# Deci-AI/super-gradients

Hardware: AMD Instinct MI355X
Metric: images/sec/node YOLO-NAS-S 640x640 train-step (higher is better)
Workload: dtype fp32 (bf16x3 MFMA); 1 GPU; YOLO-NAS-S synthetic COCO 640x640, bs=32/GPU, PPYoloELoss(TAL)+AdamW+EMA, random-init weights; global_batch=32, parallelism=dp1, conv_math=patch_bf3, conv_variant=0, bn_reduce_in_data_gradients=True, conv_tuning_entries=374, filter_planes=True

## Files before the change

### include/sgx_hip.h

```cpp
#ifndef SGX_HIP_H
#define SGX_HIP_H
#include <stdint.h>

#ifdef __cplusplus
extern "C" {
#endif

#define SGX_OK 0
#define SGX_ERR_BAD_ARG (-1)
#define SGX_ERR_UNSUPPORTED (-2)
#define SGX_ERR_HIP (-3)
#define SGX_ERR_WORKSPACE (-4)

#define SGX_ACT_NONE 0
#define SGX_ACT_RELU 1
#define SGX_ACT_SILU 2

int32_t sgx_version(void);
const char* sgx_last_error(void);

int32_t sgx_prof_enable(int32_t on);
int32_t sgx_prof_summary(int32_t cls, double* ms, double* flops, int64_t* launches);
int32_t sgx_prof_bytes(int32_t cls, double* bytes);
int32_t sgx_prof_bound_ms(int32_t cls, double peak_flops, double hbm_bytes_per_s, double* ms);
// ... 153 lines not shown
int32_t sgx_affine_act_fwd(const float* x, int64_t x_ld, const float* scale, const float* shift, const float* r1,
                           int64_t r1_ld, float a1, const float* a1_dev, const float* r2, int64_t r2_ld, float a2,
                           float* y, int64_t y_ld, int64_t M, int32_t C, int32_t act, float* partials, void* stream);
int32_t sgx_bn_bwd_reduce(const float* dy, int64_t dy_ld, const float* x, int64_t x_ld, const float* scale,
                          const float* shift, const float* save_mean, int64_t M, int32_t C, int32_t act, float* partials,
                          void* stream);
int32_t sgx_bn_bwd_finalize(const float* partials, int32_t nblk, int64_t M, int32_t C, const float* gamma,
                            const float* save_mean, const float* save_invstd, float* dgamma, float* dbeta,
                            float* coef, void* ws, int64_t ws_bytes, void* stream);
int32_t sgx_bn_bwd_apply(const float* dy, int64_t dy_ld, const float* x, int64_t x_ld, const float* scale,
                         const float* shift, const float* coef, float* dx, int64_t dx_ld, float* g_out, int64_t g_ld,
                         int64_t M, int32_t C, int32_t act, void* stream);
int64_t sgx_qarep_workspace(int32_t nblk, int32_t C);
int32_t sgx_qarep_fwd_finalize(const float* stat5, int32_t nblk, int64_t M, int32_t C, const float* bias1, const float* gamma3, const float* beta3,
                               float eps3, float mom3, float* rmean3, float* rvar3, const float* gammap, const float* betap, float epsp, float momp,
                               float* rmeanp, float* rvarp, float* cf, float* sv, void* ws, int64_t ws_bytes, void* stream);
int32_t sgx_qarep_bwd_reduce(const float* dout, int64_t d_ld, const float* y, int64_t y_ld, const float* u, int64_t u_ld, const float* cf,
                             const float* sv, int64_t M, int32_t C, int32_t act, float* partials4, void* stream);
int32_t sgx_qarep_bwd_finalize(const float* partials4, int32_t nblk, int64_t M, int32_t C, const float* gamma3, const float* gammap, const float* sv,
                               float* dgamma3, float* dgammap, float* dbetap, float* cb, void* ws, int64_t ws_bytes, void* stream);
int32_t sgx_qarep_bwd_apply(const float* dout, int64_t d_ld, const float* y, int64_t y_ld, const float* u, int64_t u_ld, const float* cf,
                            const float* sv, const float* cb, float* ds, int64_t ds_ld, float* dy, int64_t dy_ld, int64_t M, int32_t C, int32_t act,
                            void* stream);
int32_t sgx_bn_set_fused_finalize(int32_t on);
int32_t sgx_bn_get_fused_finalize(void);
int64_t sgx_dot_workspace(int64_t M, int32_t C);
int32_t sgx_dot(const float* a, int64_t a_ld, const float* b, int64_t b_ld, int64_t M, int32_t C, float scale, float* out,
                int32_t accumulate, void* ws, int64_t ws_bytes, void* stream);
int32_t sgx_axpy(const float* x, int64_t x_ld, float a, const float* a_dev, float* y, int64_t y_ld, int64_t M,
                 int32_t C, int32_t accumulate, void* stream);
int32_t sgx_relu_bwd(const float* dy, int64_t dy_ld, const float* y, int64_t y_ld, float* g, int64_t g_ld, int64_t M, int32_t C,
                     void* stream);
int32_t sgx_relu_bwd_bn_reduce(const float* dy, int64_t dy_ld, const float* y, int64_t y_ld, const float* x, int64_t x_ld,
                               const float* save_mean, float* g, int64_t g_ld, int64_t M, int32_t C, float* partials, void* stream);
int32_t sgx_dual_affine_act_fwd(const float* x1, int64_t x1_ld, const float* s1, const float* t1, const float* x2, int64_t x2_ld,
                                const float* s2, const float* t2, const float* r, int64_t r_ld, float r_scale, const float* r_scale_dev,
                                float* y, int64_t y_ld, int64_t M, int32_t C, int32_t act, void* stream);
int32_t sgx_dual_affine_act_bwd(const float* dy, int64_t dy_ld, const float* x1, int64_t x1_ld, const float* s1, const float* t1,
                                const float* x2, int64_t x2_ld, const float* s2, const float* t2, float* g, int64_t g_ld, int64_t M,
                                int32_t C, int32_t act, void* stream);
int32_t sgx_dual_affine_act_bwd_reduce(const float* dy, int64_t dy_ld, const float* x1, int64_t x1_ld, const float* s1, const float* t1,
                                       const float* mean1, const float* x2, int64_t x2_ld, const float* s2, const float* t2, const float* mean2,
                                       float* g, int64_t g_ld, int64_t M, int32_t C, int32_t act, float* partials4, void* stream);
int32_t sgx_tri_affine_act_fwd(const float* x1, int64_t x1_ld, const float* s1, const float* t1, const float* x2, int64_t x2_ld,
                               const float* s2, const float* t2, const float* x3, int64_t x3_ld, const float* s3, const float* t3,
                               const float* r, int64_t r_ld, float r_scale, const float* r_scale_dev, float* y, int64_t y_ld, int64_t M,
// ... 148 lines not shown
```

### super_gradients_amd/_lib.py

```python
import ctypes
import os
from ctypes import POINTER, c_char_p, c_float, c_int32, c_int64, c_void_p

import torch

_HERE = os.path.dirname(os.path.abspath(__file__))
LIB_PATH = os.path.join(_HERE, "csrc", "libsgx_hip.so")

_LIB = None
_TEST_HOST_MODE = False


class ConvDesc(ctypes.Structure):
    _fields_ = [(n, c_int32) for n in ("N", "H", "W", "C", "K", "R", "S", "stride", "pad", "Ho", "Wo")] + [
        (n, c_int64) for n in ("x_ld_pix", "x_ld_img", "y_ld_pix", "y_ld_img")
    ]


class LossDesc(ctypes.Structure):
    _fields_ = [
        ("B", c_int32), ("L", c_int32), ("C", c_int32), ("reg_max", c_int32), ("nmax", c_int32),
        ("use_static_assigner", c_int32), ("use_varifocal", c_int32), ("num_levels", c_int32),
        ("level_count", c_int32 * 8), ("w_cls", c_float), ("w_iou", c_float), ("w_dfl", c_float), ("sequential_assignment", c_int32),
    ]
# ... 60 lines not shown
    "sgx_conv2d_bwd_data": (_i32, [_CD, _P, _P, _P, _P, _i32, _P, _i64, _P]),
    "sgx_conv2d_transpose_weights": (_i32, [_CD, _P, _P, _i64, _P]),
    "sgx_conv2d_bwd_data_wt": (_i32, [_CD, _P, _P, _P, _P, _i32, _P]),
    "sgx_conv2d_bwd_data_stat_blocks": (_i32, [_CD, _i32]),
    "sgx_conv2d_bwd_data_wt_req": (_i32, [_CD, _P, _P, _P, _P, _i32, POINTER(BnReduceReq), _i32, _P]),
    "sgx_conv2d_bwd_data_dual_req": (_i32, [_CD, _P, _P, _P, _i64, _i64, _P, _P, _P, _i64, _i64, _f, _P, _P, _i32, POINTER(BnReduceReq), _i32, _P]),
    "sgx_conv2d_transpose_jobs": (_i32, [_CD, _P, _P, _i64, POINTER(WtransJob), _i32, POINTER(c_int32)]),
    "sgx_wtrans_batch": (_i32, [_P, _i32, _P]),
    "sgx_conv2d_fwd_dual_stat_blocks": (_i32, [_CD]),
    "sgx_conv2d_fwd_dual": (_i32, [_CD, _P, _P, _P, _P, _P, _P, _P, _P]),
    "sgx_conv2d_bwd_data_dual": (_i32, [_CD, _P, _P, _P, _i64, _i64, _P, _P, _P, _i64, _i64, _f, _P, _P, _i32, _P]),
    "sgx_qarep_prep_batch": (_i32, [_P, _i32, _P]),
    "sgx_filter_planes_bytes": (_i64, [_i32, _i32, _i32]),
    "sgx_filter_planes_batch": (_i32, [_P, _P, _i32, _P]),
    "sgx_filter_planes_invalidate": (_i32, [_P, _i32]),
    "sgx_filter_planes_scope": (_i32, [_i32]),
    "sgx_debug_set_filter_planes": (_i32, [_i32]),
    "sgx_debug_filter_planes_hits": (_i64, []),
    "sgx_qarep_workspace": (_i64, [_i32, _i32]),
    "sgx_qarep_fwd_finalize": (_i32, [_P, _i32, _i64, _i32, _P, _P, _P, _f, _f, _P, _P, _P, _P, _f, _f, _P, _P, _P, _P, _P, _i64, _P]),
    "sgx_qarep_bwd_reduce": (_i32, [_P, _i64, _P, _i64, _P, _i64, _P, _P, _i64, _i32, _i32, _P, _P]),
    "sgx_qarep_bwd_finalize": (_i32, [_P, _i32, _i64, _i32, _P, _P, _P, _P, _P, _P, _P, _P, _i64, _P]),
    "sgx_qarep_bwd_apply": (_i32, [_P, _i64, _P, _i64, _P, _i64, _P, _P, _P, _P, _i64, _P, _i64, _i64, _i32, _i32, _P]),
    "sgx_hconv2d_fwd": (_i32, [_CD, _P, _P, _P, _P, _i32, _i32, _P, _i64, _i64, _f, _P, _P]),
    "sgx_hconvT2x2_fwd": (_i32, [_i32] * 5 + [_P, _i64, _i64, _P, _P, _P, _i64, _i64, _P]),
    "sgx_hmaxpool_fwd": (_i32, [_i32] * 7 + [_P, _i64, _i64, _P, _i64, _i64, _P]),
    "sgx_hcopy": (_i32, [_P, _i64, _i64, _i32, _P, _i64, _P]),
    "sgx_himage_colsum": (_i32, [_i32, _i32, _i32, _P, _i64, _i64, _f, _P, _P]),
    "sgx_hchannel_gate": (_i32, [_i32, _i32, _i32, _P, _i64, _i64, _P, _i32, _P, _i64, _i64, _P]),
    "sgx_hupsample2x_fwd": (_i32, [_i32, _i32, _i32, _i32, _P, _i64, _i64, _P, _i64, _i64, _P]),
    "sgx_cast_f32_bf16": (_i32, [_P, _i64, _i64, _i32, _P, _i64, _i32, _P]),
    "sgx_hconv_debug_set_tile": (_i32, [_i32] * 3),
    "sgx_conv2d_bwd_weight_workspace": (_i64, [_CD]),
    "sgx_conv2d_bwd_weight": (_i32, [_CD, _P, _P, _P, _P, _P, _i64, _P]),
    "sgx_conv2d_bwd_weight_group_sizes": (_i32, [POINTER(WgradJob), _i32, POINTER(c_int64), POINTER(c_int64)]),
    "sgx_conv2d_bwd_weight_group": (_i32, [POINTER(WgradJob), _i32, _P, _i64, _P, _i64, _P]),
    "sgx_debug_set_wgrad_group": (_i32, [_i32] * 3),
    "sgx_debug_set_wgrad_loop": (_i32, [_i32]),
    "sgx_conv_set_wgrad_math": (_i32, [_i32]),
    "sgx_conv_get_wgrad_math": (_i32, []),
    "sgx_debug_set_wgrad_patch": (_i32, [_i32] * 3),
    "sgx_debug_set_bf3_min_depth": (_i32, [_i32]),
    "sgx_debug_set_nms_split": (_i32, [_i32]),
    "sgx_debug_set_nms_selection": (_i32, [_i32]),
    "sgx_debug_nms_fallback_slot": (_i32, [_P, ctypes.POINTER(ctypes.c_int64), ctypes.POINTER(ctypes.c_int32)]),
    "sgx_convT2x2_workspace": (_i64, [_i32] * 5),
# ... 214 lines not shown
```

### super_gradients_amd/csrc/bn.hip

```cpp
#include "sgx_common.h"
#include <atomic>

#define SW_THREADS 256
#define SW_MAXCG 64

struct SweepGeom {
    long M;
    int C, C4, CG, RL, nblk, rows_per_blk, ctiles;
};

extern "C" int32_t sgx_stats_blocks(int64_t M) {
    long n = (M + 63) / 64;
    if (n < 1) n = 1;
    if (n > 1024) n = 1024;
    return (int32_t)n;
}

static SweepGeom sweep_geom(long M, int C) {
    SweepGeom g;
    g.M = M;
    g.C = C;
    g.C4 = C / 4;
    g.CG = g.C4 < SW_MAXCG ? g.C4 : SW_MAXCG;
    g.RL = SW_THREADS / g.CG;
// ... 651 lines not shown
        in.a = sgx_ld4(p.x1 + row * p.x1_ld + c);
        in.b = p.x2 ? sgx_ld4(p.x2 + row * p.x2_ld + c) : make_float4(0.f, 0.f, 0.f, 0.f);
        in.d = sgx_ld4(dy + row * dy_ld + c);
        return in;
    }
    typedef DualAffineF::Cst Cst;
    __device__ Cst consts(int c) const { return p.consts(c); }
    __device__ void apply(long row, int c, const In& in, const Cst& k, float4& q0, float4& q1) const {
        (void)q0; (void)q1;
        float4 v = p.pre(k, in.a, in.b);
        sgx_st4(g + row * g_ld + c, make_float4(in.d.x * sgx_act_grad(v.x, p.act), in.d.y * sgx_act_grad(v.y, p.act),
                                                 in.d.z * sgx_act_grad(v.z, p.act), in.d.w * sgx_act_grad(v.w, p.act)));
    }
};
extern "C" int32_t sgx_dual_affine_act_bwd(const float* dy, int64_t dy_ld, const float* x1, int64_t x1_ld, const float* s1, const float* t1,
                                           const float* x2, int64_t x2_ld, const float* s2, const float* t2, float* g, int64_t g_ld, int64_t M,
                                           int32_t C, int32_t act, void* stream) {
    SGX_CHECK_ARG(dy && x1 && s1 && t1 && g, "dual_affine_act_bwd: null pointer");
    SGX_CHECK_ARG(!x2 || (s2 && t2), "dual_affine_act_bwd: second branch needs scale and shift");
    DualAffineBwdF f{DualAffineF{x1, x1_ld, s1, t1, x2, x2_ld, s2, t2, nullptr, 0, nullptr, 0, act, 1.f, nullptr}, dy, dy_ld, g, g_ld};
    return run_sweep<DualAffineBwdF, 0>(f, M, C, nullptr, stream, "dual_affine_act_bwd");
}

template <typename F, int NQ>
__global__ __launch_bounds__(SW_THREADS) void sweepq_kernel(F f, SweepGeom g, float* partials) {
    __shared__ float4 red[NQ][SW_THREADS];
    const int tid = threadIdx.x;
    const int cg = tid % g.CG, rl = tid / g.CG;
    const int c4 = blockIdx.y * g.CG + cg;
    const bool live = (rl < g.RL) && (c4 < g.C4);
    const int c = c4 * 4;
    float4 q[NQ];
#pragma unroll
    for (int k = 0; k < NQ; ++k) q[k] = make_float4(0.f, 0.f, 0.f, 0.f);
    if (live) {
        long r0 = (long)blockIdx.x * g.rows_per_blk;
        long r1 = r0 + g.rows_per_blk;
        if (r1 > g.M) r1 = g.M;
        long r = r0 + rl;
        const long st = g.RL;
        const typename F::Cst k = f.consts(c);
        for (; r + st < r1; r += 2 * st) {
            typename F::In i0 = f.load(r, c), i1 = f.load(r + st, c);
            f.apply(r, c, i0, k, q);
            f.apply(r + st, c, i1, k, q);
        }
        for (; r < r1; r += st) {
            typename F::In i0 = f.load(r, c);
            f.apply(r, c, i0, k, q);
        }
    }
    if (!partials) return;
#pragma unroll
    for (int k = 0; k < NQ; ++k) red[k][tid] = q[k];
    __syncthreads();
    if (live && rl == 0) {
#pragma unroll
        for (int k = 0; k < NQ; ++k) {
            double t[4] = {0.0, 0.0, 0.0, 0.0};
            for (int j = 0; j < g.RL; ++j) {
                const float4 a = red[k][j * g.CG + cg];
                t[0] += a.x; t[1] += a.y; t[2] += a.z; t[3] += a.w;
            }
            sgx_st4(partials + ((long)k * g.nblk + blockIdx.x) * g.C + c, make_float4((float)t[0], (float)t[1], (float)t[2], (float)t[3]));
        }
    }
}

extern "C" int64_t sgx_qarep_workspace(int32_t nblk, int32_t C) { return (int64_t)5 * cr_slices(nblk) * C * (int64_t)sizeof(double) + 256; }

__global__ void qarep_fwd_finalize_kernel(ColSrc src, long M, int C, const float* bias1, const float* g3, const float* b3, float eps3, float mom3,
                                          float* rm3, float* rv3, const float* gp, const float* bp, float epsp, float momp, float* rmp, float* rvp,
                                          float* cf, float* sv) {
    SGX_FIN_THREAD(src, C);
    double tot[5];
    col_totals<5>(src, C, c, cok, tot);
    if (!writer) return;
    const double Sy = tot[0], Syy = tot[1], Su = tot[2], Suu = tot[3], Syu = tot[4];
    const double m = (double)M, unb = M > 1 ? m / (m - 1.0) : 1.0;
    const double mean3 = Sy / m;
    double var3 = Syy / m - mean3 * mean3;
    if (var3 < 0.0) var3 = 0.0;
    const double invstd3 = 1.0 / sqrt(var3 + (double)eps3);
    const float sc3 = (g3 ? g3[c] : 1.f) * (float)invstd3;
    const float sh3 = (b3 ? b3[c] : 0.f) - (float)mean3 * sc3;
    const double mu0 = Su / m, bias = bias1 ? (double)bias1[c] : 0.0;
    double varu = Suu / m - mu0 * mu0;
// ... 55 lines not shown
    typedef QarepBwdIn In;
    __device__ In load(long r, int c) const { return b.load(r, c); }
    typedef QarepBwdBase::Cst Cst;
    __device__ Cst consts(int c) const { return b.consts(c); }
    __device__ void apply(long, int, const In& in, const Cst& k, float4 (&q)[4]) const {
        float4 g, sc, yc;
        b.terms(k, in, g, sc, yc);
        q[0].x += g.x; q[0].y += g.y; q[0].z += g.z; q[0].w += g.w;
        q[1].x += g.x * sc.x; q[1].y += g.y * sc.y; q[1].z += g.z * sc.z; q[1].w += g.w * sc.w;
        q[2].x += g.x * yc.x; q[2].y += g.y * yc.y; q[2].z += g.z * yc.z; q[2].w += g.w * yc.w;
        q[3].x += sc.x * yc.x; q[3].y += sc.y * yc.y; q[3].z += sc.z * yc.z; q[3].w += sc.w * yc.w;
    }
};
extern "C" int32_t sgx_qarep_bwd_reduce(const float* dout, int64_t d_ld, const float* y, int64_t y_ld, const float* u, int64_t u_ld, const float* cf,
                                        const float* sv, int64_t M, int32_t C, int32_t act, float* partials4, void* stream) {
    SGX_CHECK_ARG(dout && y && u && cf && sv && partials4, "qarep_bwd_reduce: null pointer");
    SGX_CHECK_ARG(M > 0 && C > 0 && C % 4 == 0, "qarep_bwd_reduce: need M>0 and C%%4==0 (C=%d)", C);
    QarepBwdReduceF f{QarepBwdBase{dout, d_ld, y, y_ld, u, u_ld, cf, sv, C, act}};
    SweepGeom g = sweep_geom(M, C);
    SGX_LAUNCH((sweepq_kernel<QarepBwdReduceF, 4>), dim3(g.nblk, g.ctiles), dim3(SW_THREADS), 0, stream, f, g, partials4);
    SGX_CHECK_LAUNCH("qarep_bwd_reduce");
    return SGX_OK;
}
__global__ void qarep_bwd_finalize_kernel(ColSrc src, long M, int C, const float* gamma3, const float* gammap, const float* sv, float* dgamma3,
                                          float* dgammap, float* dbetap, float* cb) {
    SGX_FIN_THREAD(src, C);
    double tot[4];
    col_totals<4>(src, C, c, cok, tot);
    if (!writer) return;
    const double Sg = tot[0], Sgs = tot[1], Sgy = tot[2], Ssy = tot[3];
    const double m = (double)M, invstd3 = sv[C + c], invstdp = sv[5 * C + c];
    const double gp = gammap ? (double)gammap[c] : 1.0, g3 = gamma3 ? (double)gamma3[c] : 1.0;
    if (dgammap) dgammap[c] += (float)(invstdp * Sgs);
    if (dbetap) dbetap[c] += (float)Sg;
    const double cp = gp * invstdp, kp = invstdp * invstdp * Sgs / m;
    const double Sdy = cp * (Sgy - kp * Ssy);
    if (dgamma3) dgamma3[c] += (float)(invstd3 * Sdy);
    cb[c] = (float)cp;
    const double mgd = Sg / m;
    const float mg_hi = (float)mgd;
    cb[C + c] = mg_hi;
    cb[2 * C + c] = (float)kp;
    cb[3 * C + c] = (float)(g3 * invstd3);
    cb[4 * C + c] = (float)(invstd3 * invstd3 * Sdy / m);
    cb[5 * C + c] = (float)(mgd - (double)mg_hi);
}
extern "C" int32_t sgx_qarep_bwd_finalize(const float* partials4, int32_t nblk, int64_t M, int32_t C, const float* gamma3, const float* gammap,
                                          const float* sv, float* dgamma3, float* dgammap, float* dbetap, float* cb, void* ws, int64_t ws_bytes,
                                          void* stream) {
    SGX_CHECK_ARG(partials4 && sv && cb && nblk > 0 && M > 0, "qarep_bwd_finalize: bad args");
    ColSrc src;
    int32_t rc = col_prereduce<4>(partials4, nblk, C, ws, ws_bytes, stream, &src);
    if (rc) return rc;
    SGX_LAUNCH(qarep_bwd_finalize_kernel, fin_grid(src, C), fin_block(src), 0, stream, src, (long)M, C, gamma3, gammap, sv, dgamma3, dgammap, dbetap, cb);
    SGX_CHECK_LAUNCH("qarep_bwd_finalize");
    return SGX_OK;
}
struct QarepBwdApplyF {
    QarepBwdBase b;
    const float* cb; float* ds; long ds_ld; float* dy; long dy_ld;
    typedef QarepBwdIn In;
    __device__ In load(long r, int c) const { return b.load(r, c); }
    struct Cst { QarepBwdBase::Cst t; float4 cp, mg, kp, c3, k3, ml; };
    __device__ Cst consts(int c) const {
        const int C = b.C;
        return Cst{b.consts(c), sgx_ld4(cb + c), sgx_ld4(cb + C + c), sgx_ld4(cb + 2 * C + c), sgx_ld4(cb + 3 * C + c), sgx_ld4(cb + 4 * C + c), sgx_ld4(cb + 5 * C + c)};
    }
    __device__ void apply(long r, int c, const In& in, const Cst& k, float4 (&)[1]) const {
        float4 g, sc, yc;
        b.terms(k.t, in, g, sc, yc);
        const float4 cp = k.cp, mg = k.mg, kp = k.kp, c3 = k.c3, k3 = k.k3, ml = k.ml;
        const float4 s = make_float4(cp.x * (((g.x - mg.x) - ml.x) - sc.x * kp.x), cp.y * (((g.y - mg.y) - ml.y) - sc.y * kp.y),
                                     cp.z * (((g.z - mg.z) - ml.z) - sc.z * kp.z), cp.w * (((g.w - mg.w) - ml.w) - sc.w * kp.w));
        sgx_st4(ds + r * ds_ld + c, s);
        sgx_st4(dy + r * dy_ld + c, make_float4(c3.x * (s.x - yc.x * k3.x), c3.y * (s.y - yc.y * k3.y), c3.z * (s.z - yc.z * k3.z), c3.w * (s.w - yc.w * k3.w)));
    }
};
extern "C" int32_t sgx_qarep_bwd_apply(const float* dout, int64_t d_ld, const float* y, int64_t y_ld, const float* u, int64_t u_ld, const float* cf,
// ... 327 lines not shown
```

### super_gradients_amd/kernels.py

```python
import ctypes
import functools
import os
from typing import Optional, Tuple

import torch

from . import _lib
from ._lib import ConvDesc, LossDesc, MatchDesc, NmsDesc, check, lib, ptr, stream

ACT = {None: 0, "none": 0, "relu": 1, "silu": 2}


class _Workspace:

    def __init__(self):
        self.buf = {}

    def get(self, nbytes: int, device) -> torch.Tensor:
        key = (device, stream() or 0)
        b = self.buf.get(key)
        if b is None or b.numel() < nbytes:
            b = torch.empty(max(int(nbytes * 1.25), 1 << 20), dtype=torch.uint8, device=device)
            self.buf[key] = b
        return b
# ... 16 lines not shown
    else:
        ld_pix = st[2] if st[2] >= c else (st[1] if st[1] >= c else c)
    return ld_pix, (st[0] if n > 1 else h * w * ld_pix)


def rows(t: torch.Tensor) -> Tuple[int, int]:
    ld_pix, ld_img = nhwc_strides(t)
    n, h, w, _ = t.shape
    if n > 1 and ld_img != h * w * ld_pix:
        raise _lib.SgxError("tensor rows are not uniformly strided across images")
    return n * h * w, ld_pix


_DESC_CACHE = {}


def clear_desc_cache():
    _DESC_CACHE.clear()


def clear_caches():
    clear_desc_cache()
    _TICKETS.clear()
    for f in (stats_blocks, _reduce_workspace, _qarep_workspace, _dot_workspace):
        f.cache_clear()


def conv_desc(x: torch.Tensor, K: int, R: int, S: int, stride: int, pad: int, y: Optional[torch.Tensor] = None) -> ConvDesc:
    key = (x.shape, x.stride(), K, R, S, stride, pad, None if y is None else (y.shape, y.stride()))
    d = _DESC_CACHE.get(key)
    if d is None:
        if len(_DESC_CACHE) > 65536:
            _DESC_CACHE.clear()
        d = _DESC_CACHE[key] = _conv_desc_build(x, K, R, S, stride, pad, y)
    return d


def _conv_desc_build(x, K, R, S, stride, pad, y):
    n, h, w, c = x.shape
    ho = (h + 2 * pad - R) // stride + 1
    wo = (w + 2 * pad - S) // stride + 1
    d = ConvDesc()
    d.N, d.H, d.W, d.C, d.K, d.R, d.S, d.stride, d.pad, d.Ho, d.Wo = n, h, w, c, K, R, S, stride, pad, ho, wo
    d.x_ld_pix, d.x_ld_img = nhwc_strides(x)
    if y is not None:
        if tuple(y.shape) != (n, ho, wo, K):
            raise _lib.SgxError(f"conv output shape {tuple(y.shape)} != {(n, ho, wo, K)}")
# ... 302 lines not shown
def qarep_prep_job(w1, w1p, w1pt, identity, alpha=None) -> bytes:
    K, C = w1.shape[0], w1.shape[1]
    j = _lib.QarepPrepJob()
    j.w1, j.w1p, j.w1pt, j.alpha = ptr(w1), ptr(w1p), ptr(w1pt), ptr(alpha)
    j.K, j.C, j.identity, j.pad_ = K, C, int(bool(identity)), 0
    return bytes(j)


def qarep_prep_batch(jobs_dev, njobs):
    check(lib().sgx_qarep_prep_batch(ptr(jobs_dev), int(njobs), stream()), "sgx_qarep_prep_batch")


def qarep_fwd_finalize(stat5, M, bias1, bn3, pbn):
    nblk, C = stat5.shape[1], stat5.shape[2]
    cf = torch.empty(4, C, device=stat5.device, dtype=torch.float32)
    sv = torch.empty(8, C, device=stat5.device, dtype=torch.float32)
    ws = WORKSPACE.get(_qarep_workspace(nblk, C), stat5.device)
    check(lib().sgx_qarep_fwd_finalize(ptr(stat5), nblk, M, C, ptr(bias1), ptr(bn3.weight), ptr(bn3.bias), bn3.eps, bn3.momentum, ptr(bn3.running_mean),
                                       ptr(bn3.running_var), ptr(pbn.weight), ptr(pbn.bias), pbn.eps, pbn.momentum, ptr(pbn.running_mean),
                                       ptr(pbn.running_var), ptr(cf), ptr(sv), ptr(ws), ws.numel(), stream()), "sgx_qarep_fwd_finalize")
    return cf, sv


def qarep_bwd(dout, y, u, cf, sv, bn3, pbn, act):
    M, yl = rows(y)
    C = y.shape[3]
    dl, ul = rows(dout)[1], rows(u)[1]
    a = ACT[act]
    nblk = stats_blocks(M)
    parts = torch.empty(4, nblk, C, device=y.device, dtype=torch.float32)
    check(lib().sgx_qarep_bwd_reduce(ptr(dout), dl, ptr(y), yl, ptr(u), ul, ptr(cf), ptr(sv), M, C, a, ptr(parts), stream()), "sgx_qarep_bwd_reduce")
    cb = torch.empty(6, C, device=y.device, dtype=torch.float32)
    ws = WORKSPACE.get(_qarep_workspace(nblk, C), y.device)
    check(lib().sgx_qarep_bwd_finalize(ptr(parts), nblk, M, C, ptr(bn3.weight), ptr(pbn.weight), ptr(sv), ptr(bn3.weight.grad), ptr(pbn.weight.grad),
                                       ptr(pbn.bias.grad), ptr(cb), ptr(ws), ws.numel(), stream()), "sgx_qarep_bwd_finalize")
    check(lib().sgx_qarep_bwd_apply(ptr(dout), dl, ptr(y), yl, ptr(u), ul, ptr(cf), ptr(sv), ptr(cb), ptr(u), ul, ptr(y), yl, M, C, a, stream()),
          "sgx_qarep_bwd_apply")
    return u, y


def conv2d_bwd_weight(x, dy, dw, dbias=None, stride=1, pad=0):
    K, C, R, S = dw.shape
    _chk_w(dw, K, R, S, x.shape[3])
    d = conv_desc(x, K, R, S, stride, pad, dy)
    if d.wgrad_ws is None:
        d.wgrad_ws = lib().sgx_conv2d_bwd_weight_workspace(d.ref)
    ws = WORKSPACE.get(d.wgrad_ws, x.device)
    check(lib().sgx_conv2d_bwd_weight(d.ref, ptr(x), ptr(dy), ptr(dw), ptr(dbias), ptr(ws), ws.numel(), stream()), "sgx_conv2d_bwd_weight")


_TICKETS = {}


def _ticket_buffer(n_ints: int, device) -> torch.Tensor:
    key = (device, stream() or 0)
    b = _TICKETS.get(key)
    if b is None or b.numel() < n_ints:
        b = _TICKETS[key] = torch.zeros(max(2 * int(n_ints), 1 << 16), dtype=torch.int32, device=device)
# ... 140 lines not shown


def nhwc_to_nchw(x):
    n, h, w, c = x.shape
    ld_pix, ld_img = nhwc_strides(x)
    y = torch.empty(n, c, h, w, device=x.device, dtype=torch.float32)
    check(lib().sgx_nhwc_to_nchw(n, c, h, w, ptr(x), ld_pix, ld_img, ptr(y), stream()), "sgx_nhwc_to_nchw")
    return y


@functools.lru_cache(maxsize=None)
def stats_blocks(M: int) -> int:
    return lib().sgx_stats_blocks(M)


@functools.lru_cache(maxsize=None)
def _reduce_workspace(nblk: int, C: int) -> int:
    return lib().sgx_reduce_workspace(nblk, C)


@functools.lru_cache(maxsize=None)
def _qarep_workspace(nblk: int, C: int) -> int:
    return lib().sgx_qarep_workspace(nblk, C)


@functools.lru_cache(maxsize=None)
def _dot_workspace(M: int, C: int) -> int:
    return lib().sgx_dot_workspace(M, C)


def channel_stats_partial(x):
    M, ld = rows(x)
    C = x.shape[3]
    parts = torch.empty(2, stats_blocks(M), C, device=x.device, dtype=torch.float32)
    check(lib().sgx_channel_stats_partial(ptr(x), M, C, ld, ptr(parts), stream()), "sgx_channel_stats_partial")
    return parts


def bn_finalize(parts, M, gamma, beta, eps, momentum, running_mean, running_var):
    C = parts.shape[2]
    st = torch.empty(4, C, device=parts.device, dtype=torch.float32)
    ws = WORKSPACE.get(_reduce_workspace(parts.shape[1], C), parts.device)
    p0, row = ptr(st), 4 * C
    check(lib().sgx_bn_finalize(ptr(parts), parts.shape[1], M, C, ptr(gamma), ptr(beta), eps, momentum, ptr(running_mean), ptr(running_var),
                                p0 + 2 * row, p0 + 3 * row, p0, p0 + row, ptr(ws), ws.numel(), stream()), "sgx_bn_finalize")
    return st.unbind(0)
# ... 575 lines not shown
```

### super_gradients_amd/modules/qarepvgg_block.py

```python
from torch import nn

import torch

from .. import kernels as K
from .engine import SgxBlock
from .layers import BatchNorm, ConvLayer, act_name


class _Branch(nn.Module):
    pass


class QARepVGGBlock(SgxBlock):
    def __init__(self, in_channels, out_channels, stride=1, dilation=1, groups=1, activation_type="relu", activation_kwargs=None,
                 se_type=None, se_kwargs=None, build_residual_branches=True, use_residual_connection=True, use_alpha=False,
                 use_1x1_bias=True, use_post_bn=True):
        super().__init__()
        if dilation != 1 or groups != 1:
            raise NotImplementedError("QARepVGGBlock on the HIP path: dilation=1, groups=1")
        if se_type not in (None, nn.Identity):
            raise NotImplementedError("QARepVGGBlock on the HIP path: no SE block (YOLO-NAS uses none)")
        if not (build_residual_branches and use_1x1_bias and use_post_bn):
            raise NotImplementedError("QARepVGGBlock on the HIP path implements the training form (3 branches, 1x1 bias, post-BN)")
        self.in_channels, self.out_channels, self.stride = in_channels, out_channels, stride
# ... 116 lines not shown
        self._install_fused(*self._get_equivalent_kernel_bias_for_branches())
        self.partially_fused, self.fully_fused = True, False

    def full_fusion(self):
        if self.fully_fused:
            return
        if not self.partially_fused:
            self.partial_fusion()
        pbn = self.post_bn
        k, b = self._fuse_bn_tensor(self.rbr_reparam.weight.detach(), self.rbr_reparam.bias.detach(), pbn.running_mean, pbn.running_var, pbn.weight.detach(),
                                    pbn.bias.detach(), pbn.eps)
        self._install_fused(k, b)
        self.partially_fused, self.fully_fused = False, True

    def fuse_block_residual_branches(self):
        self.partial_fusion()

    def prep_model_for_conversion(self, input_size=None, full_fusion: bool = False, **kwargs):
        if full_fusion:
            self.full_fusion()
        else:
            self.partial_fusion()

    def bwd(self, dy, dx_out=None, accumulate=False, addend=None, need_dx=True, addend2=None, addend2_scale=None, dx_req=None):
        c3, bn3, c1, pbn = self.branch_3x3.conv, self.branch_3x3.bn, self.branch_1x1, self.post_bn
        if addend2 is not None and need_dx and not (self._ctx[0] == "dual" and self.stride == 1 and K.nhwc_strides(addend2)[0] % 4 == 0):
            a, a_dev = (1.0, addend2_scale) if torch.is_tensor(addend2_scale) else (1.0 if addend2_scale is None else float(addend2_scale), None)
            dx_out = K.axpy(addend2, a=a, a_dev=a_dev, out=dx_out, accumulate=accumulate and dx_out is not None)
            accumulate, addend2 = True, None
        if self._ctx[0] == "dual":
            (_, x, y3, u, cf, sv), self._ctx = self._ctx, None
            ds, dy3 = K.qarep_bwd(dy, y3, u, cf, sv, bn3, pbn, self.act)
            c1.wgrad(x, ds, bias_grad=False)
            c3.wgrad(x, dy3)
            if not need_dx:
                return None
            return K.conv2d_bwd_data_dual(dy3, c3._w, c3._wt, ds, self._w1pt, tuple(x.shape), stride=self.stride, addend=addend, out=dx_out,
                                          accumulate=accumulate, addend2=addend2, addend2_scale=addend2_scale,
                                          reqs=dx_req if self._net.fuse_bn_reduce else None)
        (x, t3, s, sc3, sh3, m3, i3, scp, shp, mp, ip, t1), self._ctx = self._ctx, None
        ds = pbn.backward(dy, s, scp, shp, mp, ip, self.act, dx_out=s)
        ds1 = ds
        if t1 is not None:
            K.dot_sum(t1, ds, self.alpha.grad, accumulate=True)
            ds1 = K.axpy(ds, a_dev=self.alpha, out=t1)
        c1.wgrad(x, ds1, bias_grad=False)
        dt3 = bn3.backward(ds, t3, sc3, sh3, m3, i3, None, dx_out=t3)
        c3.wgrad(x, dt3)
        if not need_dx:
            return None
        shape = tuple(x.shape)
        if self.use_residual_connection:
            if dx_out is not None and K.nhwc_strides(dx_out) != K.nhwc_strides(ds):
                K.axpy(ds, out=dx_out, accumulate=accumulate)
                dx = c3.dgrad(dt3, shape, out=dx_out, accumulate=True)
# ... 6 lines not shown
```

### super_gradients_amd/training/models/detection_models/yolo_nas/yolo_stages.py

```python
import os
from functools import partial
from typing import List

import torch
from torch import nn

from ..... import kernels as K
from .....common.registry import register_detection_module
from .....modules.base_modules import BaseDetectionModule, width_multiplier
from .....modules.conv_bn_act_block import Conv
from .....modules.engine import SgxBlock
from .....modules.layers import ConvTranspose2x2, act_name
from .....modules.qarepvgg_block import QARepVGGBlock

_DALPHA_SYNC = os.environ.get("SGX_DALPHA_SYNC", "0") == "1"


def _empty(n, h, w, c, like):
    return torch.empty(n, h, w, c, device=like.device, dtype=like.dtype)


class YoloNASBottleneck(SgxBlock):

    def __init__(self, input_channels, output_channels, block_type, activation_type, shortcut: bool, use_alpha: bool, drop_path_rate: float = 0.0):
        super().__init__()
        if drop_path_rate > 0.0:
            raise NotImplementedError("drop_path inside YOLO-NAS bottlenecks is not used by the S/M/L recipes")
        self.cv1 = block_type(input_channels, output_channels, activation_type=activation_type)
        self.cv2 = block_type(output_channels, output_channels, activation_type=activation_type)
        self.add = shortcut and input_channels == output_channels
        if use_alpha:
            self.alpha = nn.Parameter(torch.tensor([1.0]), requires_grad=True)
        else:
            self.alpha = 1.0

    def on_materialize(self):
        pass

# ... 2 lines not shown

    def fwd(self, x, out=None):
        if not self.add:
            return self.cv2.fwd(self.cv1.fwd(x), out=out)
        a, a_dev = self._alpha()
        self._x = x if self.training else None
        if x.dtype == K.HALF:
            return self.cv2.fwd(self.cv1.fwd(x), out=out, post_add=x, post_scale=a_dev if a_dev is not None else a)
        if isinstance(self.cv2, QARepVGGBlock):
            return self.cv2.fwd(self.cv1.fwd(x), out=out, post_add=x, post_scale=a_dev if a_dev is not None else a)
        y = self.cv2.fwd(self.cv1.fwd(x))
        return K.affine_act(y, r1=x, a1=a, a1_dev=a_dev, out=out if out is not None else y)

    def _mid_req(self):
        r = self.cv1.bn_reduce_request() if hasattr(self.cv1, "bn_reduce_request") else None
        return [r] if r is not None else None

    def bwd(self, dz, dx_out=None, accumulate=False, addend=None, need_dx=True, dx_req=None):
        if not self.add:
            return self.cv1.bwd(self.cv2.bwd(dz, dx_req=self._mid_req()), dx_out=dx_out, accumulate=accumulate, addend=addend, need_dx=need_dx, dx_req=dx_req)
        x, self._x = self._x, None
        a, a_dev = self._alpha()
        joined = None
        if a_dev is not None:
            net = getattr(self, "_net", None)
            d_alpha = lambda: K.dot_sum(x, dz, self.alpha.grad, accumulate=True)
            if _DALPHA_SYNC and net is not None and net.side_stream is not None:
                torch.cuda.current_stream().wait_stream(net.side_stream)
            if net is not None and net.branches(32, 0, 0, True):
                joined = net.fork_branch(d_alpha, backward=True, lane=1, queues_wgrads=False)[1]
            else:
                d_alpha()
        dmid = self.cv2.bwd(dz, dx_req=self._mid_req())
        if isinstance(self.cv1, QARepVGGBlock):
            dx = self.cv1.bwd(dmid, dx_out=dx_out, accumulate=accumulate, addend=addend, addend2=dz, addend2_scale=a_dev if a_dev is not None else a,
                              dx_req=dx_req)
        else:
            if dx_out is not None:
                K.axpy(dz, a=a, a_dev=a_dev, out=dx_out, accumulate=accumulate)
                pre = dx_out
            else:
                pre = K.axpy(dz, a=a, a_dev=a_dev)
            dx = self.cv1.bwd(dmid, dx_out=pre, accumulate=True, addend=addend, dx_req=dx_req)
        if joined is not None:
            joined()
        return dx


class _BottleneckList(nn.Module):

    def __init__(self, output_intermediates, *mods):
        super().__init__()
        self.output_intermediates = output_intermediates
        for i, m in enumerate(mods):
            self.add_module(str(i), m)

# ... 250 lines not shown
```

Before: 779.9 images/s.

## Fold bottleneck alpha-gradient dot product into QARepVGG backward reduction sweep

Computes the residual alpha gradient (sum of x*dz) inside the existing QARepVGG backward reduce kernel, which already reads dz. Two extra compensated-sum (hi/lo) partial rows are added, and the finalize kernel emits the per-channel dot that a small final kernel accumulates into alpha.grad. This removes a separate full read of x and dz and the side-stream fork that used to run it. In exchange the reduce kernel reads x and carries more registers and shared memory (6 float4 slots instead of 4), and one extra tiny launch is added.

```diff
diff --git a/include/sgx_hip.h b/include/sgx_hip.h
--- a/include/sgx_hip.h
+++ b/include/sgx_hip.h
@@ -199,6 +199,12 @@
 int32_t sgx_qarep_bwd_apply(const float* dout, int64_t d_ld, const float* y, int64_t y_ld, const float* u, int64_t u_ld, const float* cf,
                             const float* sv, const float* cb, float* ds, int64_t ds_ld, float* dy, int64_t dy_ld, int64_t M, int32_t C, int32_t act,
                             void* stream);
+int64_t sgx_qarep_dot_workspace(int32_t nblk, int32_t C);
+int32_t sgx_qarep_bwd_reduce_dot(const float* dout, int64_t d_ld, const float* y, int64_t y_ld, const float* u, int64_t u_ld, const float* cf,
+                                 const float* sv, const float* x, int64_t x_ld, int64_t M, int32_t C, int32_t act, float* partials6, void* stream);
+int32_t sgx_qarep_bwd_finalize_dot(const float* partials6, int32_t nblk, int64_t M, int32_t C, const float* gamma3, const float* gammap,
+                                   const float* sv, float* dgamma3, float* dgammap, float* dbetap, float* cb, float* dalpha, void* ws,
+                                   int64_t ws_bytes, void* stream);
 int32_t sgx_bn_set_fused_finalize(int32_t on);
 int32_t sgx_bn_get_fused_finalize(void);
 int64_t sgx_dot_workspace(int64_t M, int32_t C);
diff --git a/super_gradients_amd/_lib.py b/super_gradients_amd/_lib.py
--- a/super_gradients_amd/_lib.py
+++ b/super_gradients_amd/_lib.py
@@ -106,6 +106,9 @@
     "sgx_qarep_bwd_reduce": (_i32, [_P, _i64, _P, _i64, _P, _i64, _P, _P, _i64, _i32, _i32, _P, _P]),
     "sgx_qarep_bwd_finalize": (_i32, [_P, _i32, _i64, _i32, _P, _P, _P, _P, _P, _P, _P, _P, _i64, _P]),
     "sgx_qarep_bwd_apply": (_i32, [_P, _i64, _P, _i64, _P, _i64, _P, _P, _P, _P, _i64, _P, _i64, _i64, _i32, _i32, _P]),
+    "sgx_qarep_dot_workspace": (_i64, [_i32, _i32]),
+    "sgx_qarep_bwd_reduce_dot": (_i32, [_P, _i64, _P, _i64, _P, _i64, _P, _P, _P, _i64, _i64, _i32, _i32, _P, _P]),
+    "sgx_qarep_bwd_finalize_dot": (_i32, [_P, _i32, _i64, _i32, _P, _P, _P, _P, _P, _P, _P, _P, _P, _i64, _P]),
     "sgx_hconv2d_fwd": (_i32, [_CD, _P, _P, _P, _P, _i32, _i32, _P, _i64, _i64, _f, _P, _P]),
     "sgx_hconvT2x2_fwd": (_i32, [_i32] * 5 + [_P, _i64, _i64, _P, _P, _P, _i64, _i64, _P]),
     "sgx_hmaxpool_fwd": (_i32, [_i32] * 7 + [_P, _i64, _i64, _P, _i64, _i64, _P]),
diff --git a/super_gradients_amd/csrc/bn.hip b/super_gradients_amd/csrc/bn.hip
--- a/super_gradients_amd/csrc/bn.hip
+++ b/super_gradients_amd/csrc/bn.hip
@@ -697,9 +697,12 @@
     return run_sweep<DualAffineBwdF, 0>(f, M, C, nullptr, stream, "dual_affine_act_bwd");
 }
 
+template <typename F> struct SweepqPair { static constexpr bool value = false; };
+
 template <typename F, int NQ>
 __global__ __launch_bounds__(SW_THREADS) void sweepq_kernel(F f, SweepGeom g, float* partials) {
     __shared__ float4 red[NQ][SW_THREADS];
+    constexpr int NS = SweepqPair<F>::value ? NQ - 2 : NQ;
     const int tid = threadIdx.x;
     const int cg = tid % g.CG, rl = tid / g.CG;
     const int c4 = blockIdx.y * g.CG + cg;
@@ -731,13 +734,24 @@
     __syncthreads();
     if (live && rl == 0) {
 #pragma unroll
-        for (int k = 0; k < NQ; ++k) {
+        for (int k = 0; k < NS; ++k) {
             double t[4] = {0.0, 0.0, 0.0, 0.0};
             for (int j = 0; j < g.RL; ++j) {
                 const float4 a = red[k][j * g.CG + cg];
                 t[0] += a.x; t[1] += a.y; t[2] += a.z; t[3] += a.w;
             }
             sgx_st4(partials + ((long)k * g.nblk + blockIdx.x) * g.C + c, make_float4((float)t[0], (float)t[1], (float)t[2], (float)t[3]));
+        }
+        if constexpr (SweepqPair<F>::value) {
+            double t[4] = {0.0, 0.0, 0.0, 0.0};
+            for (int j = 0; j < g.RL; ++j) {
+                const float4 a = red[NQ - 2][j * g.CG + cg], e = red[NQ - 1][j * g.CG + cg];
+                t[0] += a.x; t[0] += e.x; t[1] += a.y; t[1] += e.y; t[2] += a.z; t[2] += e.z; t[3] += a.w; t[3] += e.w;
+            }
+            const float4 hi = make_float4((float)t[0], (float)t[1], (float)t[2], (float)t[3]);
+            sgx_st4(partials + ((long)(NQ - 2) * g.nblk + blockIdx.x) * g.C + c, hi);
+            sgx_st4(partials + ((long)(NQ - 1) * g.nblk + blockIdx.x) * g.C + c,
+                    make_float4((float)(t[0] - (double)hi.x), (float)(t[1] - (double)hi.y), (float)(t[2] - (double)hi.z), (float)(t[3] - (double)hi.w)));
         }
     }
 }
@@ -839,12 +853,50 @@
     SGX_CHECK_LAUNCH("qarep_bwd_reduce");
     return SGX_OK;
 }
-__global__ void qarep_bwd_finalize_kernel(ColSrc src, long M, int C, const float* gamma3, const float* gammap, const float* sv, float* dgamma3,
-                                          float* dgammap, float* dbetap, float* cb) {
+struct QarepBwdDotIn { QarepBwdIn t; float4 x; };
+struct QarepBwdReduceDotF {
+    QarepBwdBase b;
+    const float* x; long x_ld;
+    typedef QarepBwdDotIn In;
+    __device__ In load(long r, int c) const { return In{b.load(r, c), sgx_ld4(x + r * x_ld + c)}; }
+    typedef QarepBwdBase::Cst Cst;
+    __device__ Cst consts(int c) const { return b.consts(c); }
+    __device__ void apply(long, int, const In& in, const Cst& k, float4 (&q)[6]) const {
+        float4 g, sc, yc;
+        b.terms(k, in.t, g, sc, yc);
+        q[0].x += g.x; q[0].y += g.y; q[0].z += g.z; q[0].w += g.w;
+        q[1].x += g.x * sc.x; q[1].y += g.y * sc.y; q[1].z += g.z * sc.z; q[1].w += g.w * sc.w;
+        q[2].x += g.x * yc.x; q[2].y += g.y * yc.y; q[2].z += g.z * yc.z; q[2].w += g.w * yc.w;
+        q[3].x += sc.x * yc.x; q[3].y += sc.y * yc.y; q[3].z += sc.z * yc.z; q[3].w += sc.w * yc.w;
+        auto add = [](float& s, float& e, float a, float b) {
+            const float t = fmaf(a, b, s), bp = t - s;
+            e += (s - (t - bp)) + fmaf(a, b, -bp);
+            s = t;
+        };
+        const float4 d = in.t.d, v = in.x;
+        add(q[4].x, q[5].x, v.x, d.x); add(q[4].y, q[5].y, v.y, d.y); add(q[4].z, q[5].z, v.z, d.z); add(q[4].w, q[5].w, v.w, d.w);
+    }
+};
+template <> struct SweepqPair<QarepBwdReduceDotF> { static constexpr bool value = true; };
+extern "C" int32_t sgx_qarep_bwd_reduce_dot(const float* dout, int64_t d_ld, const float* y, int64_t y_ld, const float* u, int64_t u_ld, const float* cf,
+                                            const float* sv, const float* x, int64_t x_ld, int64_t M, int32_t C, int32_t act, float* partials6,
+                                            void* stream) {
+    SGX_CHECK_ARG(dout && y && u && cf && sv && x && partials6, "qarep_bwd_reduce_dot: null pointer");
+    SGX_CHECK_ARG(M > 0 && C > 0 && C % 4 == 0, "qarep_bwd_reduce_dot: need M>0 and C%%4==0 (C=%d)", C);
+    QarepBwdReduceDotF f{QarepBwdBase{dout, d_ld, y, y_ld, u, u_ld, cf, sv, C, act}, x, x_ld};
+    SweepGeom g = sweep_geom(M, C);
+    SGX_LAUNCH((sweepq_kernel<QarepBwdReduceDotF, 6>), dim3(g.nblk, g.ctiles), dim3(SW_THREADS), 0, stream, f, g, partials6);
+    SGX_CHECK_LAUNCH("qarep_bwd_reduce_dot");
+    return SGX_OK;
+}
+template <int P>
+__device__ __forceinline__ void qarep_bwd_finalize_body(const ColSrc& src, long M, int C, const float* gamma3, const float* gammap, const float* sv,
+                                                        float* dgamma3, float* dgammap, float* dbetap, float* cb, double* dotc) {
     SGX_FIN_THREAD(src, C);
-    double tot[4];
-    col_totals<4>(src, C, c, cok, tot);
+    double tot[P];
+    col_totals<P>(src, C, c, cok, tot);
     if (!writer) return;
+    if constexpr (P == 6) dotc[c] = tot[4] + tot[5];
     const double Sg = tot[0], Sgs = tot[1], Sgy = tot[2], Ssy = tot[3];
     const double m = (double)M, invstd3 = sv[C + c], invstdp = sv[5 * C + c];
     const double gp = gammap ? (double)gammap[c] : 1.0, g3 = gamma3 ? (double)gamma3[c] : 1.0;
@@ -862,6 +914,14 @@
     cb[4 * C + c] = (float)(invstd3 * invstd3 * Sdy / m);
     cb[5 * C + c] = (float)(mgd - (double)mg_hi);
 }
+__global__ void qarep_bwd_finalize_kernel(ColSrc src, long M, int C, const float* gamma3, const float* gammap, const float* sv, float* dgamma3,
+                                          float* dgammap, float* dbetap, float* cb) {
+    qarep_bwd_finalize_body<4>(src, M, C, gamma3, gammap, sv, dgamma3, dgammap, dbetap, cb, nullptr);
+}
+__global__ void qarep_bwd_finalize_dot_kernel(ColSrc src, long M, int C, const float* gamma3, const float* gammap, const float* sv, float* dgamma3,
+                                              float* dgammap, float* dbetap, float* cb, double* dotc) {
+    qarep_bwd_finalize_body<6>(src, M, C, gamma3, gammap, sv, dgamma3, dgammap, dbetap, cb, dotc);
+}
 extern "C" int32_t sgx_qarep_bwd_finalize(const float* partials4, int32_t nblk, int64_t M, int32_t C, const float* gamma3, const float* gammap,
                                           const float* sv, float* dgamma3, float* dgammap, float* dbetap, float* cb, void* ws, int64_t ws_bytes,
                                           void* stream) {
@@ -871,6 +931,23 @@
     if (rc) return rc;
     SGX_LAUNCH(qarep_bwd_finalize_kernel, fin_grid(src, C), fin_block(src), 0, stream, src, (long)M, C, gamma3, gammap, sv, dgamma3, dgammap, dbetap, cb);
     SGX_CHECK_LAUNCH("qarep_bwd_finalize");
+    return SGX_OK;
+}
+extern "C" int64_t sgx_qarep_dot_workspace(int32_t nblk, int32_t C) { return ((int64_t)6 * cr_slices(nblk) + 1) * C * (int64_t)sizeof(double) + 256; }
+extern "C" int32_t sgx_qarep_bwd_finalize_dot(const float* partials6, int32_t nblk, int64_t M, int32_t C, const float* gamma3, const float* gammap,
+                                              const float* sv, float* dgamma3, float* dgammap, float* dbetap, float* cb, float* dalpha, void* ws,
+                                              int64_t ws_bytes, void* stream) {
+    SGX_CHECK_ARG(partials6 && sv && cb && dalpha && nblk > 0 && M > 0 && C > 0, "qarep_bwd_finalize_dot: bad args");
+    if (!ws || ws_bytes < sgx_qarep_dot_workspace(nblk, C)) SGX_FAIL(SGX_ERR_WORKSPACE, "qarep_bwd_finalize_dot: workspace too small (sgx_qarep_dot_workspace)");
+    ColSrc src;
+    int32_t rc = col_prereduce<6>(partials6, nblk, C, ws, ws_bytes, stream, &src);
+    if (rc) return rc;
+    double* dotc = (double*)ws + (long)6 * cr_slices(nblk) * C;
+    SGX_LAUNCH(qarep_bwd_finalize_dot_kernel, fin_grid(src, C), fin_block(src), 0, stream, src, (long)M, C, gamma3, gammap, sv, dgamma3, dgammap, dbetap, cb,
+               dotc);
+    SGX_CHECK_LAUNCH("qarep_bwd_finalize_dot");
+    SGX_LAUNCH(dot_final_kernel, dim3(1), dim3(256), 0, stream, (const double*)dotc, C, 1.f, dalpha, 1);
+    SGX_CHECK_LAUNCH("qarep_dalpha_final");
     return SGX_OK;
 }
 struct QarepBwdApplyF {
diff --git a/super_gradients_amd/kernels.py b/super_gradients_amd/kernels.py
--- a/super_gradients_amd/kernels.py
+++ b/super_gradients_amd/kernels.py
@@ -62,7 +62,7 @@
 def clear_caches():
     clear_desc_cache()
     _TICKETS.clear()
-    for f in (stats_blocks, _reduce_workspace, _qarep_workspace, _dot_workspace):
+    for f in (stats_blocks, _reduce_workspace, _qarep_workspace, _qarep_dot_workspace, _dot_workspace):
         f.cache_clear()
 
 
@@ -411,18 +411,29 @@
     return cf, sv
 
 
-def qarep_bwd(dout, y, u, cf, sv, bn3, pbn, act):
+def qarep_bwd(dout, y, u, cf, sv, bn3, pbn, act, dot=None):
     M, yl = rows(y)
     C = y.shape[3]
     dl, ul = rows(dout)[1], rows(u)[1]
     a = ACT[act]
     nblk = stats_blocks(M)
-    parts = torch.empty(4, nblk, C, device=y.device, dtype=torch.float32)
-    check(lib().sgx_qarep_bwd_reduce(ptr(dout), dl, ptr(y), yl, ptr(u), ul, ptr(cf), ptr(sv), M, C, a, ptr(parts), stream()), "sgx_qarep_bwd_reduce")
     cb = torch.empty(6, C, device=y.device, dtype=torch.float32)
-    ws = WORKSPACE.get(_qarep_workspace(nblk, C), y.device)
-    check(lib().sgx_qarep_bwd_finalize(ptr(parts), nblk, M, C, ptr(bn3.weight), ptr(pbn.weight), ptr(sv), ptr(bn3.weight.grad), ptr(pbn.weight.grad),
-                                       ptr(pbn.bias.grad), ptr(cb), ptr(ws), ws.numel(), stream()), "sgx_qarep_bwd_finalize")
+    if dot is not None:
+        x, alpha_grad = dot
+        if tuple(x.shape) != tuple(dout.shape):
+            raise _lib.SgxError(f"qarep_bwd: the dot operand's shape {tuple(x.shape)} is not the gradient's {tuple(dout.shape)}")
+        parts = torch.empty(6, nblk, C, device=y.device, dtype=torch.float32)
+        check(lib().sgx_qarep_bwd_reduce_dot(ptr(dout), dl, ptr(y), yl, ptr(u), ul, ptr(cf), ptr(sv), ptr(x), rows(x)[1], M, C, a, ptr(parts), stream()),
+              "sgx_qarep_bwd_reduce_dot")
+        ws = WORKSPACE.get(_qarep_dot_workspace(nblk, C), y.device)
+        check(lib().sgx_qarep_bwd_finalize_dot(ptr(parts), nblk, M, C, ptr(bn3.weight), ptr(pbn.weight), ptr(sv), ptr(bn3.weight.grad), ptr(pbn.weight.grad),
+                                               ptr(pbn.bias.grad), ptr(cb), ptr(alpha_grad), ptr(ws), ws.numel(), stream()), "sgx_qarep_bwd_finalize_dot")
+    else:
+        parts = torch.empty(4, nblk, C, device=y.device, dtype=torch.float32)
+        check(lib().sgx_qarep_bwd_reduce(ptr(dout), dl, ptr(y), yl, ptr(u), ul, ptr(cf), ptr(sv), M, C, a, ptr(parts), stream()), "sgx_qarep_bwd_reduce")
+        ws = WORKSPACE.get(_qarep_workspace(nblk, C), y.device)
+        check(lib().sgx_qarep_bwd_finalize(ptr(parts), nblk, M, C, ptr(bn3.weight), ptr(pbn.weight), ptr(sv), ptr(bn3.weight.grad), ptr(pbn.weight.grad),
+                                           ptr(pbn.bias.grad), ptr(cb), ptr(ws), ws.numel(), stream()), "sgx_qarep_bwd_finalize")
     check(lib().sgx_qarep_bwd_apply(ptr(dout), dl, ptr(y), yl, ptr(u), ul, ptr(cf), ptr(sv), ptr(cb), ptr(u), ul, ptr(y), yl, M, C, a, stream()),
           "sgx_qarep_bwd_apply")
     return u, y
@@ -609,6 +620,11 @@
 @functools.lru_cache(maxsize=None)
 def _qarep_workspace(nblk: int, C: int) -> int:
     return lib().sgx_qarep_workspace(nblk, C)
+
+
+@functools.lru_cache(maxsize=None)
+def _qarep_dot_workspace(nblk: int, C: int) -> int:
+    return lib().sgx_qarep_dot_workspace(nblk, C)
 
 
 @functools.lru_cache(maxsize=None)
diff --git a/super_gradients_amd/modules/qarepvgg_block.py b/super_gradients_amd/modules/qarepvgg_block.py
--- a/super_gradients_amd/modules/qarepvgg_block.py
+++ b/super_gradients_amd/modules/qarepvgg_block.py
@@ -162,15 +162,20 @@
         else:
             self.partial_fusion()
 
-    def bwd(self, dy, dx_out=None, accumulate=False, addend=None, need_dx=True, addend2=None, addend2_scale=None, dx_req=None):
+    def folds_dalpha(self):
+        ctx = getattr(self, "_ctx", None)
+        return ctx is not None and ctx[0] == "dual"
+
+    def bwd(self, dy, dx_out=None, accumulate=False, addend=None, need_dx=True, addend2=None, addend2_scale=None, dx_req=None, dalpha=None):
         c3, bn3, c1, pbn = self.branch_3x3.conv, self.branch_3x3.bn, self.branch_1x1, self.post_bn
+        self.dalpha_taken = dalpha is not None and self._ctx[0] == "dual"
         if addend2 is not None and need_dx and not (self._ctx[0] == "dual" and self.stride == 1 and K.nhwc_strides(addend2)[0] % 4 == 0):
             a, a_dev = (1.0, addend2_scale) if torch.is_tensor(addend2_scale) else (1.0 if addend2_scale is None else float(addend2_scale), None)
             dx_out = K.axpy(addend2, a=a, a_dev=a_dev, out=dx_out, accumulate=accumulate and dx_out is not None)
             accumulate, addend2 = True, None
         if self._ctx[0] == "dual":
             (_, x, y3, u, cf, sv), self._ctx = self._ctx, None
-            ds, dy3 = K.qarep_bwd(dy, y3, u, cf, sv, bn3, pbn, self.act)
+            ds, dy3 = K.qarep_bwd(dy, y3, u, cf, sv, bn3, pbn, self.act, dot=dalpha)
             c1.wgrad(x, ds, bias_grad=False)
             c3.wgrad(x, dy3)
             if not need_dx:
diff --git a/super_gradients_amd/training/models/detection_models/yolo_nas/yolo_stages.py b/super_gradients_amd/training/models/detection_models/yolo_nas/yolo_stages.py
--- a/super_gradients_amd/training/models/detection_models/yolo_nas/yolo_stages.py
+++ b/super_gradients_amd/training/models/detection_models/yolo_nas/yolo_stages.py
@@ -14,6 +14,7 @@
 from .....modules.qarepvgg_block import QARepVGGBlock
 
 _DALPHA_SYNC = os.environ.get("SGX_DALPHA_SYNC", "0") == "1"
+_DALPHA_IN_REDUCE = os.environ.get("SGX_DALPHA_IN_REDUCE", "1") != "0" and not _DALPHA_SYNC
 
 
 def _empty(n, h, w, c, like):
@@ -62,7 +63,10 @@
         x, self._x = self._x, None
         a, a_dev = self._alpha()
         joined = None
-        if a_dev is not None:
+        dalpha = None
+        if a_dev is not None and _DALPHA_IN_REDUCE and isinstance(self.cv2, QARepVGGBlock) and self.cv2.folds_dalpha():
+            dalpha = (x, self.alpha.grad)
+        elif a_dev is not None:
             net = getattr(self, "_net", None)
             d_alpha = lambda: K.dot_sum(x, dz, self.alpha.grad, accumulate=True)
             if _DALPHA_SYNC and net is not None and net.side_stream is not None:
@@ -71,7 +75,12 @@
                 joined = net.fork_branch(d_alpha, backward=True, lane=1, queues_wgrads=False)[1]
             else:
                 d_alpha()
-        dmid = self.cv2.bwd(dz, dx_req=self._mid_req())
+        if dalpha is not None:
+            dmid = self.cv2.bwd(dz, dx_req=self._mid_req(), dalpha=dalpha)
+            if not self.cv2.dalpha_taken:
+                K.dot_sum(x, dz, self.alpha.grad, accumulate=True)
+        else:
+            dmid = self.cv2.bwd(dz, dx_req=self._mid_req())
         if isinstance(self.cv1, QARepVGGBlock):
             dx = self.cv1.bwd(dmid, dx_out=dx_out, accumulate=accumulate, addend=addend, addend2=dz, addend2_scale=a_dev if a_dev is not None else a,
                               dx_req=dx_req)
```

Result: no change. 779.5 images/s (-0.0%).
